# wangjunchi/LLMSeg

Hardware: AMD Instinct MI355X
Metric: images/sec (1024x1024, 64-tok prompt) model_forward fwd+bwd (higher is better)
Workload: dtype bf16; 1 GPU; BASELINE.json configs[2]: synthetic 1024x1024 + random-init LLaVA-7B(Llama-7B+CLIP-L/14)/SAM-ViT-H, batch_size=2 per GPU, fwd+bwd train step (CE + align + IoP losses, LoRA r=8 dropout 0.05 on q/v + trainable embed/lm_head/text_fcs/lisa_*, frozen towers, fp32 gradient arena, AdamW step every 10 micro-steps inside the timed region, micro-step replayed from a hipGraph), 256 candidate masks, 64-token ; global_batch=2, parallelism=dp1, graph=True, valid=True

## Files before the change

### llmseg_amd/csrc/capi.cpp

```cpp
#include <hip/hip_runtime.h>
#include <stdarg.h>
#include <stdio.h>
#include <stdlib.h>
#include <algorithm>
#include <array>
#include <map>
#include <mutex>
#include <string>
#include <vector>
#include "llmseg_hip.h"

static thread_local char g_err[512] = "";

void llmseg_set_error(const char* fmt, ...) {
  va_list ap;
  va_start(ap, fmt);
  vsnprintf(g_err, sizeof(g_err), fmt, ap);
  va_end(ap);
}

extern "C" const char* llmseg_last_error(void) { return g_err; }

#include <atomic>
static std::atomic<long> g_launches{0};
// ... 73 lines not shown
    float t = 0;
    (void)hipEventElapsedTime(&t, r.a, r.b);
    ms += t;
    fl += r.flops;
    auto& c = by_class[((r.tag[3] % 10000) / 1000) * 2 + (r.tag[3] & 1)];
    c[0] += t; c[1] += r.flops; c[2] += 1;
    {
      const long S = r.tag[3] / 10000;
      auto& sp = split_by_class[((r.tag[3] % 10000) / 1000) * 2 + (r.tag[3] & 1)];
      if (S > 1) { sp[0] += 1; sp[1] += S; }
    }
    c[3] += 2.0 * ((double)r.tag[0] * r.tag[2] + (double)r.tag[1] * r.tag[2] + (double)r.tag[0] * r.tag[1]);
    auto& e = by_shape[{r.tag[0], r.tag[1], r.tag[2], r.tag[3]}];
    e[0] += t; e[1] += r.flops; e[2] += 1;
    g_pool.push_back(r);
  }
  if (getenv("LLMSEG_PROF_TABLE")) {
    std::vector<std::pair<double, std::array<long, 4>>> order;
    for (auto& kv : by_shape) order.push_back({-kv.second[0], kv.first});
    std::sort(order.begin(), order.end());
    fprintf(stderr, "%8s %8s %8s %6s %8s %10s %9s %6s\n", "M", "N", "K", "var", "calls", "total_ms", "TFLOP/s", "%time");
    const size_t top = (size_t)std::max(40, atoi(getenv("LLMSEG_PROF_TABLE")));
    for (size_t i = 0; i < order.size() && i < top; ++i) {
      auto& e = by_shape[order[i].second];
      fprintf(stderr, "%8ld %8ld %8ld %6ld %8.0f %10.2f %9.1f %6.1f\n", order[i].second[0], order[i].second[1], order[i].second[2], order[i].second[3],
              e[2], e[0], e[1] / (e[0] * 1e-3) / 1e12, 100.0 * e[0] / ms);
    }
  }
  if (total_ms) *total_ms = ms;
  if (total_flops) *total_flops = fl;
  if (launches) *launches = (int64_t)g_recs.size();
  long dom = -1;
  for (auto& kv : by_class) if (dom < 0 || kv.second[0] > by_class[dom][0]) dom = kv.first;
  static const char* names[] = {"gemm_bf16_tn_kernel<*, ...> (register staging, 128x128)", "?", "gemm_bf16_tn_glds_kernel<*, 2, 1>", "gemm_skinny_kernel<M>", "?", "?", "gemm_bf16_tn_t160_kernel (K-sliced)", "gemm_bf16_tn_pp2_kernel<*, false>",
                                "gemm_bf16_tn_pp_kernel<*, false, 4>", "gemm_bf16_tn_pp_kernel<*, false, 2>"};
  if (dom >= 0) {
    const long v = dom / 2;
    std::string nm = (v >= 0 && v < 10) ? names[v] : "?";
    const size_t star = nm.find('*');
    if (star != std::string::npos) nm.replace(star, 1, (dom & 1) ? "true" : "false");
    snprintf(g_dom_name, sizeof(g_dom_name), "%s", nm.c_str());
  } else g_dom_name[0] = 0;
  if (dom_ms) *dom_ms = dom >= 0 ? by_class[dom][0] : 0;
  if (dom_flops) *dom_flops = dom >= 0 ? by_class[dom][1] : 0;
  if (dom_launches) *dom_launches = dom >= 0 ? (int64_t)by_class[dom][2] : 0;
  g_dom_bytes = dom >= 0 ? by_class[dom][3] : 0;
  if (dom >= 0) {
    const auto& sp = split_by_class[dom];
    g_dom_info[0] = (int64_t)by_class[dom][2]; g_dom_info[1] = sp[0]; g_dom_info[2] = sp[1]; g_dom_info[3] = (int64_t)by_class[dom][2] + sp[0];
  } else g_dom_info[0] = g_dom_info[1] = g_dom_info[2] = g_dom_info[3] = 0;
  g_recs.clear();
  return LLMSEG_OK;
}
```

### llmseg_amd/csrc/gemm.hip

```cpp
#include <algorithm>
#include <cstdlib>
#include "common.h"
#include "llmseg_hip.h"

namespace {

constexpr int BN = 128, BK = 64, NT = 256;
constexpr int GROUP_M = 8;

struct GemmP {
  const bf16_t* A; const bf16_t* W; void* C;
  const bf16_t* bias; const bf16_t* gamma; const bf16_t* res;
  int M, N, K;
  long lda, ldw, ldc, ldr, sA, sW, sC, sA2, sW2, sC2;
  int batch1;
  float alpha;
  int act;
  int tiles_m, tiles_n;
  int c_vec, r_vec, b_vec;
  const bf16_t* A2; const bf16_t* W2; long lda2, ldw2;
  int group_m;
  int skew;
  int kt_total;
  int accum;
// ... 745 lines not shown
  char* cur = smem;
  char* nxt = smem + BUF;
  char* nn = smem + 2 * BUF;
  if (EXT) { PP2_ISSUE_AX(0, cur); PP_ISSUE_WX(0, cur); PP_ISSUE_WX(1, cur); PP2_ISSUE_AX(1, cur); }
  else { PP2_ISSUE_A(0, 0, cur); PP_ISSUE_W(0, 0, cur); PP_ISSUE_W(1, 0, cur); PP2_ISSUE_A(1, 0, cur); }
  PP2_ISSUE_A(0, 1, nxt); PP_ISSUE_W(0, 1, nxt); PP_ISSUE_W(1, 1, nxt); PP2_ISSUE_A(1, 1, nxt);
  PP_VMI(6);
  __builtin_amdgcn_s_barrier();
  if (wm == 1) __builtin_amdgcn_s_barrier();
  __builtin_amdgcn_sched_barrier(0);

#define PP2_READ_A P16_READ_W(wf0, 0, cur); P16_READ_W(wf1, 1, cur); P16_READ_A(0, cur)
#define PP2_MMA_A P16_MMA(wf0, 0, 0); P16_MMA(wf1, 2, 0)
#define PP2_MMA_B P16_MMA(wf1, 2, MI); P16_MMA(wf0, 0, MI)
  int t = 0;
  for (; t < nt - 2; ++t) {
    PP_PHASE(PP2_READ_A, PP2_ISSUE_A(0, t + 2, nn); PP_ISSUE_W(0, t + 2, nn), PP_NOP, PP2_MMA_A);
    PP_PHASE(P16_READ_A(MI, cur), PP_ISSUE_W(1, t + 2, nn); PP2_ISSUE_A(1, t + 2, nn), PP_VMI(6), PP2_MMA_B);
    char* const tmp = cur; cur = nxt; nxt = nn; nn = tmp;
  }
  PP_PHASE(PP2_READ_A, PP_NOP, PP_NOP, PP2_MMA_A);
  PP_PHASE(P16_READ_A(MI, cur), PP_NOP, PP_VM_0, PP2_MMA_B);
  cur = nxt;
  PP_PHASE(PP2_READ_A, PP_NOP, PP_NOP, PP2_MMA_A);
  PP_PHASE(P16_READ_A(MI, cur), PP_NOP, PP_NOP, PP2_MMA_B);
#undef PP2_READ_A
#undef PP2_MMA_A
#undef PP2_MMA_B
  if (wm == 0) __builtin_amdgcn_s_barrier();
  if constexpr (FX != FX_NONE) epilogue_fx<MI, FX>(p, Acc16<MI>{acc}, smem, wave, m0, n0, wm, wn, lane);
  else epilogue_lds<OUT_F32, MI>(p, Acc16<MI>{acc}, smem, wave, m0, n0, wm, wn, lane, bz);
}

constexpr int T160_BM = 160;
#define T160_BL(rs, dst, voff, tt) __builtin_amdgcn_raw_ptr_buffer_load_lds(rs, (lds_ptr_t)(dst), 16, voff, (int)((tt) * (BK * 2)), 0, 0)
#define T160_ISSUE_A0(tt, base) T160_BL(rsrc_a, (base) + a_lds0, a_off0, tt)
#define T160_ISSUE_A1(tt, base)                                       \
  do {                                                                \
    T160_BL(rsrc_a, (base) + a_lds1[0], a_off1[0], tt);               \
    if (two) T160_BL(rsrc_a, (base) + a_lds1[1], a_off1[1], tt);      \
  } while (0)
#define T160_ISSUE_W(h, tt, base)                                     \
  do {                                                                \
    T160_BL(rsrc_w, (base) + w_lds[h][0], w_off[h][0], tt);           \
    T160_BL(rsrc_w, (base) + w_lds[h][1], w_off[h][1], tt);           \
  } while (0)
#define T160_VM_TILE do { if (two) PP_VMI(7); else PP_VMI(6); } while (0)
#define T160_READ_A(cnt, mb0, base)                                                                                           \
  _Pragma("unroll") for (int mb = 0; mb < (cnt); ++mb) _Pragma("unroll") for (int ks = 0; ks < 2; ++ks)                     \
      af[mb][ks] = *reinterpret_cast<const bf16x8_t*>((base) + lds_off(wm * 80 + ((mb0) + mb) * 16 + frow, ks * 4 + fq))
#define T160_MMA(wfx, nb0, cnt, mb0)                                                                                          \
  _Pragma("unroll") for (int ks = 0; ks < 2; ++ks) _Pragma("unroll") for (int nb = 0; nb < 2; ++nb)                         \
      _Pragma("unroll") for (int mb = 0; mb < (cnt); ++mb)                                                                    \
          acc[(nb0) + nb][(mb0) + mb] = __builtin_amdgcn_mfma_f32_16x16x32_bf16(wfx[nb][ks], af[mb][ks], acc[(nb0) + nb][(mb0) + mb], 0, 0, 0)

__global__ __launch_bounds__(NTB, 2) void gemm_bf16_tn_t160_kernel(GemmP p) {
  constexpr int BMB = T160_BM, BNB = 256;
  constexpr int A_BYTES = BMB * BK * 2, W_BYTES = BNB * BK * 2, BUF = A_BYTES + W_BYTES;
  __shared__ __attribute__((aligned(16))) char smem[3 * BUF];
  int bid = blockIdx.x;
  const int nwg = p.tiles_m * p.tiles_n;
  {
    const int q = nwg >> 3, r = nwg & 7, xcd = bid & 7;
    const int len = q + (xcd < r ? 1 : 0);
    const int idx = ((bid >> 3) + xcd * p.skew) % len;
    bid = (xcd < r ? xcd * (q + 1) : r * (q + 1) + (xcd - r) * q) + idx;
  }
  const int per_group = p.group_m * p.tiles_n;
  const int first_m = (bid / per_group) * p.group_m;
  const int gsz = min(p.tiles_m - first_m, p.group_m);
  const int m0 = (first_m + (bid % per_group) % gsz) * BMB;
  const int n0 = ((bid % per_group) / gsz) * BNB;

  const int tid = threadIdx.x, lane = tid & 63;
  const int wave = __builtin_amdgcn_readfirstlane(tid >> 6);
  const int wm = wave >> 2, wn = wave & 3;
  const bool two = wn < 2;
  const long b1 = blockIdx.y;
  const bf16_t* __restrict__ Ag = p.A + b1 * p.sA;
  const bf16_t* __restrict__ Wg = p.W + b1 * p.sW;
  const __amdgpu_buffer_rsrc_t rsrc_a = __builtin_amdgcn_make_buffer_rsrc(const_cast<bf16_t*>(Ag + (long)m0 * p.lda), 0, 0x7fffffff, 0x00020000);
  const __amdgpu_buffer_rsrc_t rsrc_w = __builtin_amdgcn_make_buffer_rsrc(const_cast<bf16_t*>(Wg + (long)n0 * p.ldw), 0, 0x7fffffff, 0x00020000);
  auto a_src = [&](int ra0) { const int ra = ra0 + (lane >> 3); return (int)(((long)min(ra, p.M - 1 - m0) * p.lda + (((lane & 7) ^ ((ra >> 1) & 7)) << 3)) * 2); };
  const int ra_a0 = wm * 80 + wn * 8;
  const int j1 = 8 + 2 * wm + (wn & 1);
  const int ra_a1[2] = {(wave / 6) * 80 + 32 + (wave % 6) * 8, (j1 / 6) * 80 + 32 + (j1 % 6) * 8};
  const int a_lds0 = ra_a0 * 128, a_off0 = a_src(ra_a0);
  const int a_lds1[2] = {ra_a1[0] * 128, ra_a1[1] * 128};
  const int a_off1[2] = {a_src(ra_a1[0]), a_src(ra_a1[1])};
  int w_off[2][2], w_lds[2][2];
#pragma unroll
  for (int h = 0; h < 2; ++h) {
#pragma unroll
    for (int i = 0; i < 2; ++i) {
      const int rw0 = PP_WROW0(h, i), rw = rw0 + (lane >> 3);
      w_lds[h][i] = A_BYTES + rw0 * 128;
      w_off[h][i] = (int)(((long)min(rw, p.N - 1 - n0) * p.ldw + (((lane & 7) ^ ((rw >> 1) & 7)) << 3)) * 2);
    }
  }
  int nt = p.K / BK;
  nt = min(nt, p.kt_total - (int)b1 * nt);

  f32x4_t acc[4][5];
#pragma unroll
  for (int nb = 0; nb < 4; ++nb)
#pragma unroll
    for (int mb = 0; mb < 5; ++mb) acc[nb][mb] = f32x4_t{0.f, 0.f, 0.f, 0.f};
  bf16x8_t af[3][2], wf0[2][2], wf1[2][2];
  const int frow = lane & 15, fq = lane >> 4;
  const int wrow0 = wn * 64, wrow1 = wrow0 + 32;

  char* cur = smem;
  char* nxt = smem + BUF;
  char* nn = smem + 2 * BUF;
  T160_ISSUE_A0(0, cur); T160_ISSUE_W(0, 0, cur); T160_ISSUE_W(1, 0, cur); T160_ISSUE_A1(0, cur);
  T160_ISSUE_A0(1, nxt); T160_ISSUE_W(0, 1, nxt); T160_ISSUE_W(1, 1, nxt); T160_ISSUE_A1(1, nxt);
  T160_VM_TILE;
  __builtin_amdgcn_s_barrier();
  if (wm == 1) __builtin_amdgcn_s_barrier();
  __builtin_amdgcn_sched_barrier(0);

#define T160_RD_A P16_READ_W(wf0, 0, cur); P16_READ_W(wf1, 1, cur); T160_READ_A(2, 0, cur)
#define T160_RD_B T160_READ_A(3, 2, cur)
#define T160_MMA_A T160_MMA(wf0, 0, 2, 0); T160_MMA(wf1, 2, 2, 0)
#define T160_MMA_B T160_MMA(wf1, 2, 3, 2); T160_MMA(wf0, 0, 3, 2)
  int t = 0;
  for (; t < nt - 2; ++t) {
    PP_PHASE(T160_RD_A, T160_ISSUE_A0(t + 2, nn); T160_ISSUE_W(0, t + 2, nn), PP_NOP, T160_MMA_A);
    PP_PHASE(T160_RD_B, T160_ISSUE_W(1, t + 2, nn); T160_ISSUE_A1(t + 2, nn), T160_VM_TILE, T160_MMA_B);
    char* const tmp = cur; cur = nxt; nxt = nn; nn = tmp;
  }
  PP_PHASE(T160_RD_A, PP_NOP, PP_NOP, T160_MMA_A);
  PP_PHASE(T160_RD_B, PP_NOP, PP_VMI(0), T160_MMA_B);
  cur = nxt;
  PP_PHASE(T160_RD_A, PP_NOP, PP_NOP, T160_MMA_A);
  PP_PHASE(T160_RD_B, PP_NOP, PP_NOP, T160_MMA_B);
#undef T160_RD_A
#undef T160_RD_B
#undef T160_MMA_A
#undef T160_MMA_B
  if (wm == 0) __builtin_amdgcn_s_barrier();

  float* slab = reinterpret_cast<float*>(smem) + wave * (32 * 64);
  const int r15 = lane & 15, q4 = lane >> 4;
  const int c = lane & 15, rsub = lane >> 4;
  const int n = n0 + wn * 64 + c * 4;
  const int mw = m0 + wm * 80;
  float* cbase = reinterpret_cast<float*>(p.C) + b1 * p.sC;
#pragma unroll
  for (int i = 0; i < 3; ++i) {
    const int nh = i < 2 ? 2 : 1;
#pragma unroll
    for (int h = 0; h < nh; ++h)
#pragma unroll
      for (int nb = 0; nb < 4; ++nb) {
        const int row = h * 16 + r15, chunk = nb * 4 + q4;
        *reinterpret_cast<float4*>(slab + row * 64 + ((chunk ^ (row & 15)) << 2)) =
            make_float4(acc[nb][2 * i + h][0], acc[nb][2 * i + h][1], acc[nb][2 * i + h][2], acc[nb][2 * i + h][3]);
      }
#pragma unroll
    for (int it = 0; it < 4 * nh; ++it) {
      const int row = it * 4 + rsub;
      const float4 a4 = *reinterpret_cast<const float4*>(slab + row * 64 + ((c ^ (row & 15)) << 2));
      const int m = mw + i * 32 + row;
      if (m >= p.M || n >= p.N) continue;
      *reinterpret_cast<float4*>(cbase + (long)m * p.ldc + n) =
          make_float4(fmaf(a4.x, p.alpha, 0.f), fmaf(a4.y, p.alpha, 0.f), fmaf(a4.z, p.alpha, 0.f), fmaf(a4.w, p.alpha, 0.f));
    }
  }
}
#undef T160_BL
#undef T160_ISSUE_A0
#undef T160_ISSUE_A1
#undef T160_ISSUE_W
#undef T160_VM_TILE
// ... 275 lines not shown
    const int c = threadIdx.x + 256 * i;
    if (c < nch) {
      const int n = c * 8;
      const float* sp = slab + m * p.N + n;
      float4 a0 = *reinterpret_cast<const float4*>(sp), a1 = *reinterpret_cast<const float4*>(sp + 4);
      for (int s2 = 1; s2 < S; ++s2) {
        const float4 b0 = *reinterpret_cast<const float4*>(sp + s2 * slab_sz), b1 = *reinterpret_cast<const float4*>(sp + s2 * slab_sz + 4);
        a0.x += b0.x; a0.y += b0.y; a0.z += b0.z; a0.w += b0.w;
        a1.x += b1.x; a1.y += b1.y; a1.z += b1.z; a1.w += b1.w;
      }
      const float v[8] = {a0.x * p.alpha, a0.y * p.alpha, a0.z * p.alpha, a0.w * p.alpha, a1.x * p.alpha, a1.y * p.alpha, a1.z * p.alpha, a1.w * p.alpha};
      const uint4 g = pack8(v);
      *reinterpret_cast<uint4*>(reinterpret_cast<bf16_t*>(p.C) + m * p.ldc + n) = g;
      float of[8], df[8];
      unpack8(*reinterpret_cast<const uint4*>(O + m * ldo + n), of);
      unpack8(g, df);
      float part = 0.f;
#pragma unroll
      for (int e = 0; e < 8; ++e) part = fmaf(of[e], df[e], part);
#pragma unroll
      for (int mm = 8; mm >= 1; mm >>= 1) part += __shfl_xor(part, mm, 64);
      if ((c & 15) == 0) delta[(b * heads + (c >> 4)) * T + q] = part;
    }
  }
}

enum GemmKernel {
  K_REG = 0,
  K_GLDS = 2,
  K_AUTO = 5,
  K_PP256 = 8,
  K_PP128 = 9,
  K_T160 = 10,
};
inline bool is_pp(GemmKernel k) { return k == K_PP256 || k == K_PP128 || k == K_T160; }
inline int pp_rows(GemmKernel k) { return k == K_PP256 ? 256 : k == K_T160 ? T160_BM : 128; }
inline GemmKernel kernel_of_knob(int v) { return v == K_REG || v == K_GLDS || is_pp((GemmKernel)v) ? (GemmKernel)v : K_AUTO; }

template <bool OUT_F32, bool EXT, int FX = FX_NONE>
void launch_pp(GemmKernel k, const GemmP& p, dim3 grid, hipStream_t s) {
  if (k == K_PP256) LL_LAUNCH_KERNEL((gemm_bf16_tn_pp_kernel<OUT_F32, EXT, FX>), grid, dim3(NTB), 0, s, p);
  else LL_LAUNCH_KERNEL((gemm_bf16_tn_pp2_kernel<OUT_F32, EXT, FX>), grid, dim3(NTB), 0, s, p);
}

enum TailKind {
  TAIL_NORM,
  TAIL_NB,
  TAIL_DL,
  TAIL_FX,
};
struct GemmTail { TailKind kind; const llmseg_gemm_args* req; bool done; };

}

void llmseg_prof_begin(hipStream_t s);
void llmseg_prof_end(hipStream_t s, double flops);
void llmseg_prof_tag(long a, long b, long c, long d);

static int g_gemm_variant = K_AUTO, g_gemm_skew = 13, g_gemm_split = 0;
static const bool g_gemm_t160 = getenv("LLMSEG_GEMM_NO_T160") == nullptr;
static const int g_gemm_rsplit = getenv("LLMSEG_GEMM_NO_RSPLIT") ? 0 : 1;
static int num_cus() {
  static int n = [] { int dev = 0, v = 0; (void)hipGetDevice(&dev); (void)hipDeviceGetAttribute(&v, hipDeviceAttributeMultiprocessorCount, dev); return v > 0 ? v : 256; }();
  return n;
}
extern "C" int llmseg_gemm_set_variant(int v) {
  g_gemm_variant = v & 15;
  if ((v >> 4) & 15) g_gemm_skew = ((v >> 4) & 15) - 1;
  g_gemm_split = (v >> 8) & 31;
  return LLMSEG_OK;
}

namespace {
struct GemmPlan { GemmKernel kernel; int split; double us; };
constexpr double T160_KT_US = 1.13;
inline double pp_cost(long M, long N, int nt, int bm, int S, long ncu, bool f32out) {
  const long tiles = ((M + bm - 1) / bm) * ((N + 255) / 256);
  const long rounds = (tiles * S + ncu - 1) / ncu;
  const int q = (nt + S - 1) / S;
  const double it = bm == 256 ? 1.7 : bm == 160 ? T160_KT_US : 1.0, fix = (bm == 256 ? 7.0 : 4.5) + ((S > 1 || f32out) ? 1.0 : 0.0);
  double eff_rounds = (double)rounds;
  if (S == 1) {
    const long full = tiles / ncu, rem = tiles - full * ncu;
    eff_rounds = (double)full + (rem ? 0.5 + 0.5 * (double)rem / (double)ncu : 0.0);
  }
  double us = eff_rounds * (q * it + fix);
  if (S > 1) us += 2.5 + ((double)(S + 1) * M * N * 4.0) / 4.0e6;
  return us;
}
inline double glds_cost(long M, long N, int nt, long ncu) {
  const long tiles = ((M + 127) / 128) * ((N + 127) / 128);
  const long full = tiles / (4 * ncu), rem = tiles - full * 4 * ncu;
  double us = (double)full * (nt * 2.4 + 4.0);
  if (rem > 0) { const double w = (double)((rem + ncu - 1) / ncu); us += nt * std::max(1.3, 0.6 * w) + 4.0; }
  return us;
}
inline bool split_ok(int nt, int S) {
  if (S <= 1) return S == 1;
  const int q = (nt + S - 1) / S;
  return q >= 2 && nt - (S - 1) * q >= 2;
}
}

static int gemm_dispatch(const llmseg_gemm_args* a, void* stream, GemmTail* tail);

extern "C" int llmseg_norm(const void* x, const void* w, const void* b, void* y, int64_t rows, int64_t cols, int64_t ldx, int64_t ldy, float eps, int rms,
                           const int32_t* row_map, void* stream);

extern "C" int llmseg_rope(void* x, const float* cos, const float* sin, int64_t rows, int64_t T, int32_t heads, int32_t head_dim, int64_t ld, void* stream);
extern "C" int llmseg_swiglu(const void* gu, void* out, int64_t rows, int64_t I, int64_t ldgu, int64_t ldo, void* stream);
extern "C" __attribute__((visibility("hidden"))) int llmseg_swiglu_bwd_ld(const void* gu, const void* dout, void* dgu, int64_t rows, int64_t I, int64_t ld_dout, void* stream);

static const bool g_fx_off = getenv("LLMSEG_GEMM_NO_FX") != nullptr;

static int gemm_fx(const llmseg_gemm_args* a, void* stream) {
  LL_CHECK(a->fx >= 1 && a->fx <= 3, "gemm: unknown fx %d", a->fx);
  LL_CHECK(!a->out_f32 && a->batch <= 1 && a->batch2 <= 1 && a->alpha == 1.f && !a->bias && !a->gamma && !a->residual && a->act == LLMSEG_ACT_NONE && !a->norm_out &&
               !a->trans_a && !a->trans_w && !a->accumulate, "gemm: fx needs a plain bf16 product (batch 1, alpha 1, no bias / activation / gamma / residual / norm_out)");
  if (a->fx == LLMSEG_FX_ROPE) {
    LL_CHECK(a->fx_cos && a->fx_sin && a->fx_T > 0 && a->fx_cols > 0 && (a->fx_cols % 128) == 0 && a->fx_cols <= a->N && (a->ldc & 3) == 0 &&
                 ((((uintptr_t)a->fx_cos) | ((uintptr_t)a->fx_sin)) & 15) == 0 && (((uintptr_t)a->C) & 7) == 0,
// ... 104 lines not shown
  LL_CHECK((((uintptr_t)a->A) & 15) == 0 && (((uintptr_t)a->W) & 15) == 0, "gemm: A/W must be 16-byte aligned");
  LL_CHECK(((a->strideA | a->strideW | a->strideA2 | a->strideW2) & 7) == 0, "gemm: batch strides of A/W must be multiples of 8");
  LL_CHECK(!a->accumulate || a->out_f32, "gemm: accumulate needs fp32 output");
  const int esz = a->out_f32 ? 4 : 2;
  GemmP p;
  p.A = (const bf16_t*)a->A; p.W = (const bf16_t*)a->W; p.C = a->C;
  p.bias = (const bf16_t*)a->bias; p.gamma = (const bf16_t*)a->gamma; p.res = (const bf16_t*)a->residual;
  p.M = (int)a->M; p.N = (int)a->N; p.K = (int)a->K;
  p.lda = a->lda; p.ldw = a->ldw; p.ldc = a->ldc; p.ldr = a->residual ? a->ldr : 0;
  const long batch1 = a->batch > 0 ? a->batch : 1, batch2 = a->batch2 > 0 ? a->batch2 : 1;
  const long batch = batch1 * batch2;
  p.batch1 = (int)batch1;
  p.sA = a->strideA; p.sW = a->strideW; p.sC = a->strideC;
  p.sA2 = a->strideA2; p.sW2 = a->strideW2; p.sC2 = a->strideC2;
  p.alpha = a->alpha; p.act = a->act;
  p.kt_total = 0; p.k_split_total = 0; p.accum = a->accumulate ? 1 : 0;
  p.fx = 0; p.fx_T = a->fx_T; p.fx_cols = (int)a->fx_cols; p.fx_I = a->fx == LLMSEG_FX_SWIGLU ? (int)(a->N / 2) : (int)a->N;
  p.fx_cos = a->fx_cos; p.fx_sin = a->fx_sin; p.fx_out = (bf16_t*)a->fx_out; p.fx_in = (const bf16_t*)a->fx_in; p.fx_ld = a->fx_ld;
  p.c_vec = ((((uintptr_t)a->C) % (4 * esz)) == 0 && (a->ldc & 3) == 0 && ((a->strideC | a->strideC2) & 3) == 0) ? 1 : 0;
  p.r_vec = (p.res && (((uintptr_t)p.res) & 7) == 0 && (p.ldr & 3) == 0 && ((a->strideC | a->strideC2) & 3) == 0) ? 1 : 0;
  p.b_vec = ((p.bias == nullptr || (((uintptr_t)p.bias) & 7) == 0) && (p.gamma == nullptr || (((uintptr_t)p.gamma) & 7) == 0)) ? 1 : 0;

  p.skew = g_gemm_skew;
  p.A2 = (const bf16_t*)a->A2; p.W2 = (const bf16_t*)a->W2; p.lda2 = a->lda2; p.ldw2 = a->ldw2;
  static const int group_m_env = getenv("LLMSEG_GEMM_GROUP_M") ? atoi(getenv("LLMSEG_GEMM_GROUP_M")) : 0;
  const int nt = p.K / BK;
  const long ncu = num_cus();
  GemmKernel kernel = (p.K % BK == 0 && !ta && !tw) ? kernel_of_knob(g_gemm_variant) : K_REG;
  if ((kernel == K_PP256 || kernel == K_PP128) && nt < (a->A2 ? 1 : 2)) kernel = K_GLDS;
  if (kernel == K_T160 && nt < 2) kernel = K_GLDS;
  const bool can_split = batch == 1 && (p.N & 3) == 0 && (p.ldc & 3) == 0 && a->workspace != nullptr &&
                         (((uintptr_t)a->workspace) & 15) == 0 && (!p.res || (p.ldr & 3) == 0);
  auto ws_fits = [&](int S) { return (double)(S + (a->A2 ? 1 : 0)) * p.M * p.N * 4.0 <= (double)a->workspace_bytes; };
  int split = 1;
  if (kernel == K_AUTO) {
    GemmPlan best{K_GLDS, 1, glds_cost(p.M, p.N, nt, ncu) * (double)batch};
    if (nt >= (a->A2 ? 1 : 2)) {
      const bool t160 = g_gemm_t160 && !a->fx && !a->residual;
      for (const GemmKernel k : {K_PP256, K_PP128, K_T160}) {
        if (k == K_T160 && !t160) continue;
        const int bm = pp_rows(k);
        for (int S = k == K_T160 ? 2 : 1; S <= 16; ++S) {
          if (S > 1 && (!can_split || !split_ok(nt, S) || !ws_fits(S))) continue;
          if (S > 1 && ((p.M + bm - 1) / bm) * ((p.N + 255) / 256) * S > ncu) break;
          const double us = pp_cost(p.M, p.N, nt, bm, S, ncu, a->out_f32 != 0) * (double)batch;
          if (us < best.us * 0.97 || (us < best.us && S == 1)) best = GemmPlan{k, S, us};
        }
      }
    }
    kernel = best.kernel; split = best.split;
  } else if (kernel == K_PP256 || kernel == K_PP128) {
    split = g_gemm_split > 1 ? g_gemm_split : 1;
    if (split > 1) LL_CHECK(can_split && split_ok(nt, split) && ws_fits(split), "gemm: forced split-K %d not possible for this call", split);
  } else if (kernel == K_T160) {
    split = g_gemm_split;
    LL_CHECK(split > 1 && can_split && split_ok(nt, split) && ws_fits(split), "gemm: variant 10 (160 x 256, K-sliced) needs a forced split-K count >= 2 that is possible for this call (got %d)", split);
  }
  if (p.A2) {
    LL_CHECK(p.W2 && batch == 1 && !ta && !tw && (p.lda2 & 7) == 0 && (p.ldw2 & 7) == 0 && p.lda2 >= 64 && p.ldw2 >= 64 &&
                 (((uintptr_t)p.A2 | (uintptr_t)p.W2) & 15) == 0, "gemm: bad extension operands (A2 [M][64], W2 [N][64], 16-byte aligned rows)");
    LL_CHECK(!a->out_f32, "gemm: extension operands need bf16 output");
    if (is_pp(kernel) && split > 1) {
      llmseg_gemm_args g2 = *a;
      g2.A = a->A2; g2.W = a->W2; g2.lda = a->lda2; g2.ldw = a->ldw2; g2.K = 64; g2.A2 = g2.W2 = nullptr;
      g2.bias = g2.gamma = g2.residual = nullptr; g2.alpha = 1.f; g2.act = LLMSEG_ACT_NONE; g2.out_f32 = 1; g2.accumulate = 0;
      g2.C = (float*)a->workspace + (long)split * p.M * p.N; g2.ldc = p.N; g2.workspace = nullptr; g2.workspace_bytes = 0;
      const int rc = gemm_dispatch(&g2, stream, nullptr);
      if (rc != LLMSEG_OK) return rc;
    } else if (!is_pp(kernel)) {
      LL_CHECK(a->act == LLMSEG_ACT_NONE && !a->gamma, "gemm: extension operands on this shape need a linear epilogue");
      llmseg_gemm_args g1 = *a, g2 = *a;
      g1.A2 = g1.W2 = nullptr;
      int rc = gemm_dispatch(&g1, stream, nullptr);
      if (rc != LLMSEG_OK) return rc;
      g2.A = a->A2; g2.W = a->W2; g2.lda = a->lda2; g2.ldw = a->ldw2; g2.K = 64; g2.bias = nullptr; g2.residual = a->C; g2.ldr = a->ldc;
      g2.A2 = g2.W2 = nullptr;
      return gemm_dispatch(&g2, stream, nullptr);
    }
  }
  p.a_norm_w = (const bf16_t*)a->a_norm_w; p.a_norm_eps = a->a_norm_eps; p.a_swiglu = a->a_swiglu;
  const bool a_xform = p.a_norm_w || p.a_swiglu;
  LL_CHECK(!a_xform || (p.M <= 8 && !ta && !tw && batch == 1 && !p.A2 && (p.K & 7) == 0 && !(p.a_norm_w && p.a_swiglu) &&
                        (!p.a_norm_w || (((uintptr_t)p.a_norm_w) & 15) == 0) && (!p.a_swiglu || p.lda >= 2 * p.K)),
           "gemm: A-row transforms (a_norm_w / a_swiglu) are decode-step fusions of the M <= 8 route");
  if (p.M <= 8 && !ta && !tw && batch == 1 && !p.A2 && (p.K & 7) == 0 && (g_gemm_variant == K_AUTO || a_xform)) {
    hipStream_t s = (hipStream_t)stream;
    llmseg_prof_begin(s);
    llmseg_prof_tag(p.M, p.N, p.K, 3000 + (p.res ? 20 : 0) + p.act * 2 + (a->out_f32 ? 1 : 0));
    static const int sk_env = getenv("LLMSEG_SKINNY_SK") ? atoi(getenv("LLMSEG_SKINNY_SK")) : 1;
    const bool sk = sk_env == 2 ? p.K >= 2048 : (sk_env && p.N <= 8192 && p.K >= 2048);
    const dim3 grid((unsigned)(sk ? (p.N + 3) / 4 : (p.N + 15) / 16));
    const int of = a->out_f32 ? 1 : 0;
#define LL_SKINNY_(AT, SKV)                                                                                   \
    do {                                                                                                      \
      if (p.M == 1) LL_LAUNCH_KERNEL((gemm_skinny_kernel<1, AT, SKV>), grid, dim3(256), 0, s, p, of);      \
      else if (p.M == 2) LL_LAUNCH_KERNEL((gemm_skinny_kernel<2, AT, SKV>), grid, dim3(256), 0, s, p, of); \
      else if (p.M <= 4) LL_LAUNCH_KERNEL((gemm_skinny_kernel<4, AT, SKV>), grid, dim3(256), 0, s, p, of); \
      else LL_LAUNCH_KERNEL((gemm_skinny_kernel<8, AT, SKV>), grid, dim3(256), 0, s, p, of);               \
    } while (0)
#define LL_SKINNY(AT) do { if (sk) LL_SKINNY_(AT, true); else LL_SKINNY_(AT, false); } while (0)
    if (p.a_norm_w) LL_SKINNY(1); else if (p.a_swiglu) LL_SKINNY(2); else LL_SKINNY(0);
#undef LL_SKINNY_
#undef LL_SKINNY
    llmseg_prof_end(s, 2.0 * (double)a->M * (double)a->N * (double)a->K);
    LL_LAUNCH_CHECK("gemm_skinny");
    return LLMSEG_OK;
  }
  const bool pp = is_pp(kernel);
  const int bm = pp ? pp_rows(kernel) : 128, bn = pp ? 256 : BN;
  p.tiles_m = (p.M + bm - 1) / bm; p.tiles_n = (p.N + bn - 1) / bn;
  p.group_m = group_m_env > 0 ? group_m_env : (p.tiles_m <= 32 ? ((p.tiles_n > 16 && p.tiles_m > 8) ? 8 : p.tiles_m) : 4);
  hipStream_t s = (hipStream_t)stream;
  llmseg_prof_begin(s);
  llmseg_prof_tag(p.M, p.N, p.K, (kernel == K_PP128 ? 7 : kernel == K_T160 ? 6 : (int)kernel) * 1000 + (ta ? 200 : 0) + (tw ? 100 : 0) + (p.res ? 20 : 0) + p.act * 2 + (a->out_f32 ? 1 : 0) + 40 * (batch > 1) +
                  10000 * (split > 1 ? split : 0));
  const bool f = a->out_f32 != 0;
  if (kernel == K_REG && batch2 == 1 && (p.N & 3) == 0 && (p.ldc & 3) == 0 && a->workspace != nullptr && (((uintptr_t)a->workspace) & 15) == 0 &&
      (!p.res || ((p.ldr & 3) == 0 && batch == 1)) && ((p.sC & 3) == 0 || batch == 1) && g_gemm_rsplit) {
    const long tiles = (long)p.tiles_m * p.tiles_n * batch;
    const int ntr = (p.K + BK - 1) / BK;
    int S = (tiles * 4 <= ncu && ntr >= 8) ? (int)std::min<long>({(long)ncu / std::max<long>(tiles, 1), (long)ntr / 2, 32L}) : 1;
    while (S > 1 && (double)S * batch * p.M * p.N * 4.0 > (double)a->workspace_bytes) --S;
    if (S > 1) {
      const int q = (ntr + S - 1) / S;
      S = (ntr + q - 1) / q;
    }
    if (S > 1) {
      const int q = (ntr + S - 1) / S;
      GemmP ps = p;
      ps.K = q * BK; ps.k_split_total = p.K; ps.batch1 = S;
      ps.sA = ta ? (long)q * BK * p.lda : (long)q * BK; ps.sW = tw ? (long)q * BK * p.ldw : (long)q * BK;
      ps.sA2 = p.sA; ps.sW2 = p.sW;
      ps.C = a->workspace; ps.ldc = p.N; ps.sC = (long)p.M * p.N; ps.sC2 = (long)S * p.M * p.N;
      ps.bias = ps.gamma = ps.res = nullptr; ps.ldr = 0; ps.alpha = 1.f; ps.act = LLMSEG_ACT_NONE; ps.accum = 0;
      ps.c_vec = 1; ps.r_vec = 0; ps.b_vec = 1;
      const dim3 grid(p.tiles_m * p.tiles_n, (unsigned)(S * batch));
      const int key = (ta ? 2 : 0) | (tw ? 1 : 0);
      switch (key) {
        case 0: LL_LAUNCH_KERNEL((gemm_bf16_tn_kernel<true, false, false>), grid, dim3(NT), 0, s, ps); break;
        case 1: LL_LAUNCH_KERNEL((gemm_bf16_tn_kernel<true, false, true>), grid, dim3(NT), 0, s, ps); break;
        case 2: LL_LAUNCH_KERNEL((gemm_bf16_tn_kernel<true, true, false>), grid, dim3(NT), 0, s, ps); break;
        default: LL_LAUNCH_KERNEL((gemm_bf16_tn_kernel<true, true, true>), grid, dim3(NT), 0, s, ps); break;
      }
      const long total4 = (long)p.M * (p.N >> 2);
      const unsigned rg = (unsigned)std::min<long>((total4 + 255) / 256, 4096);
      LL_LAUNCH_KERNEL(splitk_reduce_kernel, dim3(rg, (unsigned)batch), dim3(256), 0, s, p, (const float*)a->workspace, S, f ? 1 : 0);
      llmseg_prof_end(s, 2.0 * (double)a->M * (double)a->N * (double)a->K * (double)batch);
      LL_LAUNCH_CHECK("gemm_bf16_tn (K-sliced)");
      return LLMSEG_OK;
    }
  }
  if (pp && split > 1) {
    GemmP ps = p;
    const int q = (nt + split - 1) / split;
    ps.K = q * BK; ps.kt_total = nt; ps.batch1 = split;
    ps.sA = ps.sW = (long)q * BK; ps.sA2 = ps.sW2 = ps.sC2 = 0;
    ps.C = a->workspace; ps.ldc = p.N; ps.sC = (long)p.M * p.N;
    ps.bias = ps.gamma = ps.res = nullptr; ps.ldr = 0; ps.alpha = 1.f; ps.act = LLMSEG_ACT_NONE; ps.accum = 0;
    ps.c_vec = 1; ps.r_vec = 0; ps.b_vec = 1; ps.A2 = ps.W2 = nullptr;
    dim3 grid(p.tiles_m * p.tiles_n, (unsigned)split);
    if (kernel == K_T160) LL_LAUNCH_KERNEL(gemm_bf16_tn_t160_kernel, grid, dim3(NTB), 0, s, ps);
    else launch_pp<true, false>(kernel, ps, grid, s);
    const float* slabs = (const float*)a->workspace;
    const int S2 = split + (p.A2 ? 1 : 0);
    const int cpt = ((p.N >> 3) + 255) / 256;
    const llmseg_gemm_args* r = tail ? tail->req : nullptr;
    static const long wg_max_rows = getenv("LLMSEG_NORM_WG_MAX") ? atol(getenv("LLMSEG_NORM_WG_MAX")) : 2048;
    const bool fuse_norm = tail && tail->kind == TAIL_NORM && !f && p.alpha == 1.f && !p.bias && !p.gamma && p.act == LLMSEG_ACT_NONE && p.M >= 64 && p.M < wg_max_rows &&
                           p.N >= 2048 && p.N <= 8192 && (p.N & 7) == 0 && (p.ldc & 7) == 0 && (!p.res || (p.ldr & 7) == 0) && (r->ldn & 7) == 0 &&
                           ((((uintptr_t)p.C) | ((uintptr_t)p.res) | ((uintptr_t)r->norm_w) | ((uintptr_t)r->norm_out)) & 15) == 0;
    const bool fuse_nb = tail && tail->kind == TAIL_NB && !f && p.alpha == 1.f && !p.bias && !p.gamma && !p.res && p.act == LLMSEG_ACT_NONE && p.M >= 64 && p.N >= 2048 &&
                         p.N <= 8192 && (p.N & 7) == 0;
    const bool fuse_dl = tail && tail->kind == TAIL_DL && !f && !p.bias && !p.gamma && !p.res && p.act == LLMSEG_ACT_NONE && p.N <= 8192 && (p.N & 127) == 0 && (p.ldc & 7) == 0;
    if (fuse_dl) {
#define LL_RDL(C) LL_LAUNCH_KERNEL(splitk_reduce_delta_kernel<C>, dim3((unsigned)p.M), dim3(256), 0, s, p, slabs, S2, (const bf16_t*)r->dl_o, (long)r->dl_ldo, r->dl_out, \
                                   (int)r->dl_heads, (int)r->dl_T)
      if (cpt <= 1) LL_RDL(1); else if (cpt <= 2) LL_RDL(2); else LL_RDL(4);
#undef LL_RDL
    } else if (fuse_nb) {
      const int rc = llmseg_reduce_lora_normbwd(slabs, S2, p.M, p.N, r->nb_x, r->nb_w, r->C, r->nb_eps, r->nb_rms, r->nb_dres, (void*)r->nb_lora_t, r->nb_lora_ldt, r->nb_lora_w0,
                                                r->nb_lora_w1, r->nb_lora_alpha, (const llmseg_dropout*)r->nb_lora_drop, r->nb_lora_part, r->nb_lora_S, r->nb_lora_scale,
                                                r->nb_lora_zero, stream);
      if (rc != LLMSEG_OK) return rc;
    } else if (fuse_norm) {
#define LL_RNORM(C) LL_LAUNCH_KERNEL(splitk_reduce_rmsnorm_kernel<C>, dim3((unsigned)p.M), dim3(256), 0, s, p, slabs, S2, (const bf16_t*)r->norm_w, r->norm_eps, \
                                     (bf16_t*)r->norm_out, (long)r->ldn)
      if (cpt <= 1) LL_RNORM(1); else if (cpt <= 2) LL_RNORM(2); else LL_RNORM(4);
#undef LL_RNORM
    } else {
      const long total4 = (long)p.M * (p.N >> 2);
      const unsigned rg = (unsigned)std::min<long>((total4 + 255) / 256, 4096);
      LL_LAUNCH_KERNEL(splitk_reduce_kernel, dim3(rg), dim3(256), 0, s, p, slabs, S2, f ? 1 : 0);
    }
    if (fuse_dl || fuse_nb || fuse_norm) tail->done = true;
// ... 40 lines not shown
```

Measured before the change: 52.84 images/s.

## Add direct (non-split) 160-row tile GEMM variant with fused epilogue

Templates the 160x256 t160 GEMM kernel on a DIRECT flag. With the flag set, the kernel swaps operand roles so the 160-row tile runs over N and the 256 side over M, and writes bf16 output directly through an LDS-staged epilogue that applies bias, activation, gamma and residual. The planner picks this variant when its cost model beats the other candidates, so eligible GEMMs skip the split-K fp32 workspace and the separate reduce kernel. In exchange there is a new cost model with hand-fitted constants, an extra template instantiation, and a single-K-tile path that has to handle the pipeline prologue and epilogue correctly.

```diff
diff --git a/llmseg_amd/csrc/capi.cpp b/llmseg_amd/csrc/capi.cpp
--- a/llmseg_amd/csrc/capi.cpp
+++ b/llmseg_amd/csrc/capi.cpp
@@ -129,7 +129,7 @@
   if (launches) *launches = (int64_t)g_recs.size();
   long dom = -1;
   for (auto& kv : by_class) if (dom < 0 || kv.second[0] > by_class[dom][0]) dom = kv.first;
-  static const char* names[] = {"gemm_bf16_tn_kernel<*, ...> (register staging, 128x128)", "?", "gemm_bf16_tn_glds_kernel<*, 2, 1>", "gemm_skinny_kernel<M>", "?", "?", "gemm_bf16_tn_t160_kernel (K-sliced)", "gemm_bf16_tn_pp2_kernel<*, false>",
+  static const char* names[] = {"gemm_bf16_tn_kernel<*, ...> (register staging, 128x128)", "?", "gemm_bf16_tn_glds_kernel<*, 2, 1>", "gemm_skinny_kernel<M>", "gemm_bf16_tn_t160_kernel<true> (direct, 256 x 160 of C)", "?", "gemm_bf16_tn_t160_kernel<false> (K-sliced)", "gemm_bf16_tn_pp2_kernel<*, false>",
                                 "gemm_bf16_tn_pp_kernel<*, false, 4>", "gemm_bf16_tn_pp_kernel<*, false, 2>"};
   if (dom >= 0) {
     const long v = dom / 2;
diff --git a/llmseg_amd/csrc/gemm.hip b/llmseg_amd/csrc/gemm.hip
--- a/llmseg_amd/csrc/gemm.hip
+++ b/llmseg_amd/csrc/gemm.hip
@@ -801,6 +801,70 @@
   else epilogue_lds<OUT_F32, MI>(p, Acc16<MI>{acc}, smem, wave, m0, n0, wm, wn, lane, bz);
 }
 
+constexpr int T160D_LD = 84;
+template <int ACT>
+__device__ __forceinline__ void epilogue_t160d(const GemmP& p, const f32x4_t (&acc)[4][5], float* slab, int cm0, int cn0, int lane) {
+  const int r15 = lane & 15, q4 = lane >> 4;
+  float bs[5], gm[5];
+#pragma unroll
+  for (int mb = 0; mb < 5; ++mb) {
+    const int n = cn0 + 16 * mb + r15;
+    bs[mb] = p.bias ? bf2f(p.bias[n]) : 0.f;
+    gm[mb] = p.gamma ? bf2f(p.gamma[n]) : 1.f;
+  }
+  const float alpha = p.alpha;
+  const bool has_gamma = p.gamma != nullptr;
+  bf16_t* C = reinterpret_cast<bf16_t*>(p.C);
+#pragma unroll
+  for (int pass = 0; pass < 2; ++pass) {
+    uint4 rpre[5];
+    if (p.res) {
+#pragma unroll
+      for (int it = 0; it < 5; ++it) {
+        const int pi = it * 64 + lane, row = pi / 10, pc = pi - row * 10;
+        const int m = min(cm0 + pass * 32 + row, p.M - 1);
+        rpre[it] = *reinterpret_cast<const uint4*>(p.res + (long)m * p.ldr + cn0 + pc * 8);
+      }
+    }
+#pragma unroll
+    for (int h = 0; h < 2; ++h)
+#pragma unroll
+      for (int mb = 0; mb < 5; ++mb) {
+        const f32x4_t a = acc[2 * pass + h][mb];
+        float v[4] = {fmaf(a[0], alpha, bs[mb]), fmaf(a[1], alpha, bs[mb]), fmaf(a[2], alpha, bs[mb]), fmaf(a[3], alpha, bs[mb])};
+        if (ACT == LLMSEG_ACT_GELU) {
+          const f32x2_t g0 = gelu2(f32x2_t{v[0], v[1]}), g1 = gelu2(f32x2_t{v[2], v[3]});
+          v[0] = g0.x; v[1] = g0.y; v[2] = g1.x; v[3] = g1.y;
+        } else if (ACT != LLMSEG_ACT_NONE) {
+#pragma unroll
+          for (int e = 0; e < 4; ++e) v[e] = apply_act(v[e], ACT);
+        }
+        if (has_gamma) {
+#pragma unroll
+          for (int e = 0; e < 4; ++e) v[e] *= gm[mb];
+        }
+#pragma unroll
+        for (int e = 0; e < 4; ++e) slab[(h * 16 + 4 * q4 + e) * T160D_LD + 16 * mb + r15] = v[e];
+      }
+#pragma unroll
+    for (int it = 0; it < 5; ++it) {
+      const int pi = it * 64 + lane, row = pi / 10, pc = pi - row * 10;
+      const float4 x0 = *reinterpret_cast<const float4*>(slab + row * T160D_LD + pc * 8);
+      const float4 x1 = *reinterpret_cast<const float4*>(slab + row * T160D_LD + pc * 8 + 4);
+      const int m = cm0 + pass * 32 + row;
+      if (m >= p.M) continue;
+      float v[8] = {x0.x, x0.y, x0.z, x0.w, x1.x, x1.y, x1.z, x1.w};
+      if (p.res) {
+        const uint32_t rr[4] = {rpre[it].x, rpre[it].y, rpre[it].z, rpre[it].w};
+#pragma unroll
+        for (int e = 0; e < 4; ++e) { v[2 * e] += __uint_as_float(rr[e] << 16); v[2 * e + 1] += __uint_as_float(rr[e] & 0xffff0000u); }
+      }
+      *reinterpret_cast<uint4*>(C + (long)m * p.ldc + cn0 + pc * 8) = make_uint4(pack2bf(v[0], v[1]), pack2bf(v[2], v[3]), pack2bf(v[4], v[5]), pack2bf(v[6], v[7]));
+    }
+  }
+}
+
+
 constexpr int T160_BM = 160;
 #define T160_BL(rs, dst, voff, tt) __builtin_amdgcn_raw_ptr_buffer_load_lds(rs, (lds_ptr_t)(dst), 16, voff, (int)((tt) * (BK * 2)), 0, 0)
 #define T160_ISSUE_A0(tt, base) T160_BL(rsrc_a, (base) + a_lds0, a_off0, tt)
@@ -823,6 +887,7 @@
       _Pragma("unroll") for (int mb = 0; mb < (cnt); ++mb)                                                                    \
           acc[(nb0) + nb][(mb0) + mb] = __builtin_amdgcn_mfma_f32_16x16x32_bf16(wfx[nb][ks], af[mb][ks], acc[(nb0) + nb][(mb0) + mb], 0, 0, 0)
 
+template <bool DIRECT>
 __global__ __launch_bounds__(NTB, 2) void gemm_bf16_tn_t160_kernel(GemmP p) {
   constexpr int BMB = T160_BM, BNB = 256;
   constexpr int A_BYTES = BMB * BK * 2, W_BYTES = BNB * BK * 2, BUF = A_BYTES + W_BYTES;
@@ -845,12 +910,14 @@
   const int wave = __builtin_amdgcn_readfirstlane(tid >> 6);
   const int wm = wave >> 2, wn = wave & 3;
   const bool two = wn < 2;
-  const long b1 = blockIdx.y;
-  const bf16_t* __restrict__ Ag = p.A + b1 * p.sA;
-  const bf16_t* __restrict__ Wg = p.W + b1 * p.sW;
-  const __amdgpu_buffer_rsrc_t rsrc_a = __builtin_amdgcn_make_buffer_rsrc(const_cast<bf16_t*>(Ag + (long)m0 * p.lda), 0, 0x7fffffff, 0x00020000);
-  const __amdgpu_buffer_rsrc_t rsrc_w = __builtin_amdgcn_make_buffer_rsrc(const_cast<bf16_t*>(Wg + (long)n0 * p.ldw), 0, 0x7fffffff, 0x00020000);
-  auto a_src = [&](int ra0) { const int ra = ra0 + (lane >> 3); return (int)(((long)min(ra, p.M - 1 - m0) * p.lda + (((lane & 7) ^ ((ra >> 1) & 7)) << 3)) * 2); };
+  const long b1 = DIRECT ? 0 : blockIdx.y;
+  const bf16_t* __restrict__ Ag = DIRECT ? p.W : p.A + b1 * p.sA;
+  const bf16_t* __restrict__ Wg = DIRECT ? p.A : p.W + b1 * p.sW;
+  const long ld160 = DIRECT ? p.ldw : p.lda, ld256 = DIRECT ? p.lda : p.ldw;
+  const int rows160 = DIRECT ? p.N : p.M, rows256 = DIRECT ? p.M : p.N;
+  const __amdgpu_buffer_rsrc_t rsrc_a = __builtin_amdgcn_make_buffer_rsrc(const_cast<bf16_t*>(Ag + (long)m0 * ld160), 0, 0x7fffffff, 0x00020000);
+  const __amdgpu_buffer_rsrc_t rsrc_w = __builtin_amdgcn_make_buffer_rsrc(const_cast<bf16_t*>(Wg + (long)n0 * ld256), 0, 0x7fffffff, 0x00020000);
+  auto a_src = [&](int ra0) { const int ra = ra0 + (lane >> 3); return (int)(((long)min(ra, rows160 - 1 - m0) * ld160 + (((lane & 7) ^ ((ra >> 1) & 7)) << 3)) * 2); };
   const int ra_a0 = wm * 80 + wn * 8;
   const int j1 = 8 + 2 * wm + (wn & 1);
   const int ra_a1[2] = {(wave / 6) * 80 + 32 + (wave % 6) * 8, (j1 / 6) * 80 + 32 + (j1 % 6) * 8};
@@ -864,11 +931,12 @@
     for (int i = 0; i < 2; ++i) {
       const int rw0 = PP_WROW0(h, i), rw = rw0 + (lane >> 3);
       w_lds[h][i] = A_BYTES + rw0 * 128;
-      w_off[h][i] = (int)(((long)min(rw, p.N - 1 - n0) * p.ldw + (((lane & 7) ^ ((rw >> 1) & 7)) << 3)) * 2);
+      w_off[h][i] = (int)(((long)min(rw, rows256 - 1 - n0) * ld256 + (((lane & 7) ^ ((rw >> 1) & 7)) << 3)) * 2);
     }
   }
   int nt = p.K / BK;
-  nt = min(nt, p.kt_total - (int)b1 * nt);
+  if (!DIRECT) nt = min(nt, p.kt_total - (int)b1 * nt);
+  const bool pair = !DIRECT || nt > 1;
 
   f32x4_t acc[4][5];
 #pragma unroll
@@ -883,8 +951,10 @@
   char* nxt = smem + BUF;
   char* nn = smem + 2 * BUF;
   T160_ISSUE_A0(0, cur); T160_ISSUE_W(0, 0, cur); T160_ISSUE_W(1, 0, cur); T160_ISSUE_A1(0, cur);
-  T160_ISSUE_A0(1, nxt); T160_ISSUE_W(0, 1, nxt); T160_ISSUE_W(1, 1, nxt); T160_ISSUE_A1(1, nxt);
-  T160_VM_TILE;
+  if (pair) {
+    T160_ISSUE_A0(1, nxt); T160_ISSUE_W(0, 1, nxt); T160_ISSUE_W(1, 1, nxt); T160_ISSUE_A1(1, nxt);
+    T160_VM_TILE;
+  } else PP_VMI(0);
   __builtin_amdgcn_s_barrier();
   if (wm == 1) __builtin_amdgcn_s_barrier();
   __builtin_amdgcn_sched_barrier(0);
@@ -899,9 +969,11 @@
     PP_PHASE(T160_RD_B, T160_ISSUE_W(1, t + 2, nn); T160_ISSUE_A1(t + 2, nn), T160_VM_TILE, T160_MMA_B);
     char* const tmp = cur; cur = nxt; nxt = nn; nn = tmp;
   }
-  PP_PHASE(T160_RD_A, PP_NOP, PP_NOP, T160_MMA_A);
-  PP_PHASE(T160_RD_B, PP_NOP, PP_VMI(0), T160_MMA_B);
-  cur = nxt;
+  if (pair) {
+    PP_PHASE(T160_RD_A, PP_NOP, PP_NOP, T160_MMA_A);
+    PP_PHASE(T160_RD_B, PP_NOP, PP_VMI(0), T160_MMA_B);
+    cur = nxt;
+  }
   PP_PHASE(T160_RD_A, PP_NOP, PP_NOP, T160_MMA_A);
   PP_PHASE(T160_RD_B, PP_NOP, PP_NOP, T160_MMA_B);
 #undef T160_RD_A
@@ -910,6 +982,19 @@
 #undef T160_MMA_B
   if (wm == 0) __builtin_amdgcn_s_barrier();
 
+  if constexpr (DIRECT) {
+    float* tslab = reinterpret_cast<float*>(smem) + wave * (32 * T160D_LD);
+    const int cm0 = n0 + wn * 64, cn0 = m0 + wm * 80;
+    switch (p.act) {
+      case LLMSEG_ACT_NONE: epilogue_t160d<LLMSEG_ACT_NONE>(p, acc, tslab, cm0, cn0, lane); break;
+      case LLMSEG_ACT_GELU: epilogue_t160d<LLMSEG_ACT_GELU>(p, acc, tslab, cm0, cn0, lane); break;
+      case LLMSEG_ACT_QUICKGELU: epilogue_t160d<LLMSEG_ACT_QUICKGELU>(p, acc, tslab, cm0, cn0, lane); break;
+      case LLMSEG_ACT_SILU: epilogue_t160d<LLMSEG_ACT_SILU>(p, acc, tslab, cm0, cn0, lane); break;
+      case LLMSEG_ACT_RELU: epilogue_t160d<LLMSEG_ACT_RELU>(p, acc, tslab, cm0, cn0, lane); break;
+      default: epilogue_t160d<LLMSEG_ACT_SIGMOID>(p, acc, tslab, cm0, cn0, lane); break;
+    }
+    return;
+  }
   float* slab = reinterpret_cast<float*>(smem) + wave * (32 * 64);
   const int r15 = lane & 15, q4 = lane >> 4;
   const int c = lane & 15, rsub = lane >> 4;
@@ -1251,10 +1336,11 @@
   K_PP256 = 8,
   K_PP128 = 9,
   K_T160 = 10,
+  K_T160D = 11,
 };
 inline bool is_pp(GemmKernel k) { return k == K_PP256 || k == K_PP128 || k == K_T160; }
 inline int pp_rows(GemmKernel k) { return k == K_PP256 ? 256 : k == K_T160 ? T160_BM : 128; }
-inline GemmKernel kernel_of_knob(int v) { return v == K_REG || v == K_GLDS || is_pp((GemmKernel)v) ? (GemmKernel)v : K_AUTO; }
+inline GemmKernel kernel_of_knob(int v) { return v == K_REG || v == K_GLDS || v == K_T160D || is_pp((GemmKernel)v) ? (GemmKernel)v : K_AUTO; }
 
 template <bool OUT_F32, bool EXT, int FX = FX_NONE>
 void launch_pp(GemmKernel k, const GemmP& p, dim3 grid, hipStream_t s) {
@@ -1278,6 +1364,7 @@
 
 static int g_gemm_variant = K_AUTO, g_gemm_skew = 13, g_gemm_split = 0;
 static const bool g_gemm_t160 = getenv("LLMSEG_GEMM_NO_T160") == nullptr;
+static const bool g_gemm_t160d = getenv("LLMSEG_GEMM_NO_T160D") == nullptr;
 static const int g_gemm_rsplit = getenv("LLMSEG_GEMM_NO_RSPLIT") ? 0 : 1;
 static int num_cus() {
   static int n = [] { int dev = 0, v = 0; (void)hipGetDevice(&dev); (void)hipDeviceGetAttribute(&v, hipDeviceAttributeMultiprocessorCount, dev); return v > 0 ? v : 256; }();
@@ -1306,6 +1393,11 @@
   double us = eff_rounds * (q * it + fix);
   if (S > 1) us += 2.5 + ((double)(S + 1) * M * N * 4.0) / 4.0e6;
   return us;
+}
+constexpr double T160D_KT_US = 1.35, T160D_FIX_US = 9.4;
+inline double t160d_cost(long M, long N, int nt, long ncu) {
+  const long tiles = ((M + 255) / 256) * (N / T160_BM);
+  return (double)((tiles + ncu - 1) / ncu) * (nt * T160D_KT_US + T160D_FIX_US);
 }
 inline double glds_cost(long M, long N, int nt, long ncu) {
   const long tiles = ((M + 127) / 128) * ((N + 127) / 128);
@@ -1476,6 +1568,8 @@
   const bool can_split = batch == 1 && (p.N & 3) == 0 && (p.ldc & 3) == 0 && a->workspace != nullptr &&
                          (((uintptr_t)a->workspace) & 15) == 0 && (!p.res || (p.ldr & 3) == 0);
   auto ws_fits = [&](int S) { return (double)(S + (a->A2 ? 1 : 0)) * p.M * p.N * 4.0 <= (double)a->workspace_bytes; };
+  const bool t160d_ok = p.K % BK == 0 && !ta && !tw && p.N % T160_BM == 0 && !a->out_f32 && !p.A2 && batch == 1 && !tail && !a->fx && (p.ldc & 7) == 0 &&
+                        (((uintptr_t)p.C) & 15) == 0 && (!p.res || ((p.ldr & 7) == 0 && (((uintptr_t)p.res) & 15) == 0));
   int split = 1;
   if (kernel == K_AUTO) {
     GemmPlan best{K_GLDS, 1, glds_cost(p.M, p.N, nt, ncu) * (double)batch};
@@ -1492,7 +1586,13 @@
         }
       }
     }
+    if (g_gemm_t160d && t160d_ok) {
+      const double us = t160d_cost(p.M, p.N, nt, ncu);
+      if (us < best.us) best = GemmPlan{K_T160D, 1, us};
+    }
     kernel = best.kernel; split = best.split;
+  } else if (kernel == K_T160D) {
+    LL_CHECK(t160d_ok, "gemm: variant 11 (direct 160-row tile) needs N %% 160 == 0, K %% 64 == 0, bf16 output, no extension / fused tail / batch, 16-byte aligned C and residual rows");
   } else if (kernel == K_PP256 || kernel == K_PP128) {
     split = g_gemm_split > 1 ? g_gemm_split : 1;
     if (split > 1) LL_CHECK(can_split && split_ok(nt, split) && ws_fits(split), "gemm: forced split-K %d not possible for this call", split);
@@ -1556,7 +1656,7 @@
   p.group_m = group_m_env > 0 ? group_m_env : (p.tiles_m <= 32 ? ((p.tiles_n > 16 && p.tiles_m > 8) ? 8 : p.tiles_m) : 4);
   hipStream_t s = (hipStream_t)stream;
   llmseg_prof_begin(s);
-  llmseg_prof_tag(p.M, p.N, p.K, (kernel == K_PP128 ? 7 : kernel == K_T160 ? 6 : (int)kernel) * 1000 + (ta ? 200 : 0) + (tw ? 100 : 0) + (p.res ? 20 : 0) + p.act * 2 + (a->out_f32 ? 1 : 0) + 40 * (batch > 1) +
+  llmseg_prof_tag(p.M, p.N, p.K, (kernel == K_PP128 ? 7 : kernel == K_T160 ? 6 : kernel == K_T160D ? 4 : (int)kernel) * 1000 + (ta ? 200 : 0) + (tw ? 100 : 0) + (p.res ? 20 : 0) + p.act * 2 + (a->out_f32 ? 1 : 0) + 40 * (batch > 1) +
                   10000 * (split > 1 ? split : 0));
   const bool f = a->out_f32 != 0;
   if (kernel == K_REG && batch2 == 1 && (p.N & 3) == 0 && (p.ldc & 3) == 0 && a->workspace != nullptr && (((uintptr_t)a->workspace) & 15) == 0 &&
@@ -1594,7 +1694,12 @@
       return LLMSEG_OK;
     }
   }
-  if (pp && split > 1) {
+  if (kernel == K_T160D) {
+    GemmP pd = p;
+    pd.tiles_m = p.N / T160_BM; pd.tiles_n = (p.M + 255) / 256;
+    pd.group_m = group_m_env > 0 ? group_m_env : std::min(pd.tiles_m, 8);
+    LL_LAUNCH_KERNEL(gemm_bf16_tn_t160_kernel<true>, dim3((unsigned)(pd.tiles_m * pd.tiles_n)), dim3(NTB), 0, s, pd);
+  } else if (pp && split > 1) {
     GemmP ps = p;
     const int q = (nt + split - 1) / split;
     ps.K = q * BK; ps.kt_total = nt; ps.batch1 = split;
@@ -1603,7 +1708,7 @@
     ps.bias = ps.gamma = ps.res = nullptr; ps.ldr = 0; ps.alpha = 1.f; ps.act = LLMSEG_ACT_NONE; ps.accum = 0;
     ps.c_vec = 1; ps.r_vec = 0; ps.b_vec = 1; ps.A2 = ps.W2 = nullptr;
     dim3 grid(p.tiles_m * p.tiles_n, (unsigned)split);
-    if (kernel == K_T160) LL_LAUNCH_KERNEL(gemm_bf16_tn_t160_kernel, grid, dim3(NTB), 0, s, ps);
+    if (kernel == K_T160) LL_LAUNCH_KERNEL(gemm_bf16_tn_t160_kernel<false>, grid, dim3(NTB), 0, s, ps);
     else launch_pp<true, false>(kernel, ps, grid, s);
     const float* slabs = (const float*)a->workspace;
     const int S2 = split + (p.A2 ? 1 : 0);
```

After: 52.82 images/s (median of 2 runs). Within noise of the previous version (-0.0%).
